# KELVIN-ASU/Lightweight-Multi-Modal-Scene-Understanding-via-Knowledge-Distillation

Hardware: AMD Instinct MI355X
Metric: PandaSet 2-class KD training frames/sec (higher is better)
Workload: dtype f32; 1 GPU; KD step: concat-fusion teacher fwd (eval) -> weighted-fusion student fwd/bwd (train BN), CE + T^2*KL(T=4) + feature-MSE, fused AdamW; random-init weights; teacher_fusion=concat, student_fusion=weighted, image=3x256x256, points_per_frame=80000, bev_grid=64x64, num_classes=2, per_gpu_batch=256, global_batch=256, parallelism=dp1

## Files before the change

### include/kd_hip.h

```cpp
#ifndef KD_HIP_H
#define KD_HIP_H
#include <stddef.h>
#include <stdint.h>

#ifdef __cplusplus
extern "C" {
#endif

#define KD_ACT_NONE 0
#define KD_ACT_RELU 1
#define KD_ACT_RELU6 2

int kd_version(void);
const char* kd_arch(void);
const char* kd_last_error_string(void);

int kd_set_gemm_split(int on);
int64_t kd_pwconv_stat_rows(int64_t M);
int64_t kd_pwconv_stat_rows_for(int64_t M, int K, int N, int pro, int epi, int with_addend);
int kd_set_gemm_stream(int mode);
int kd_pwconv_gemm(const float* A, int64_t lda, const float* A2, int64_t lda2, int pro, int pro_act,
                   const float* p0, const float* p1, const float* p2, const float* p3, const float* p4,
                   const float* W, const float* bias, float* C, int64_t ldc, const float* addend,
                   int64_t ldadd, int epi, const float* X, int64_t ldx, const float* esc, const float* esh,
// ... 149 lines not shown
int64_t kd_lidar_seg_stat_rows(int64_t ncells);
int kd_lidar_seg_max_bwd(const float* y, const float* sc, const float* sh, int act, const float* grid,
                         const float* dout, const float* mean, const float* invstd, const int* seg_start,
                         const int* perm, const int* row_of_point, float* G, float* partial, int64_t P,
                         int64_t ncells, int C, void* stream);
int kd_lidar_compact(const float* pts, float* out_pts, int* out_cell, int* counter, int B, int64_t N, int H, int W,
                     float x0, float x1, float y0, float y1, void* stream);
int kd_lidar_scatter_max_idx_fwd(const float* y, const float* sc, const float* sh, int act, const int* cell_idx,
                                 float* grid, int64_t P, int C, int64_t ncells, const int* p_dev, void* stream);

int kd_bilinear_accum_fwd(const float* in, const float* sc, const float* sh, int act, float* out, int accumulate,
                          int B, int Hi, int Wi, int Ho, int Wo, int C, void* stream);
int kd_bilinear_sum_fwd(const float* in0, const float* sc0, const float* sh0, int act0, int H0, int W0, const float* in1,
                        const float* sc1, const float* sh1, int act1, int H1, int W1, const float* in2, const float* sc2,
                        const float* sh2, int act2, int H2, int W2, float* out, int B, int Ho, int Wo, int C, void* stream);
int kd_bilinear_bwd(const float* dout, const float* in, const float* sc, const float* sh, int act,
                    const float* mean, const float* invstd, float* gin, float* partial, int B, int Hi, int Wi,
                    int Ho, int Wo, int C, void* stream);
int kd_weighted_fuse_fwd(const float* cat, const float* sc, const float* sh, const float* hraw, const float* w2,
                         const float* b2, float* out, float* wts, int64_t M, int C, void* stream);
size_t kd_weighted_fuse_bwd_ws_bytes(int64_t M, int C);
int kd_weighted_fuse_bwd(const float* dout, const float* cat, const float* sc, const float* sh, const float* hraw,
                         const float* w2, const float* wts, float* dcat, float* gh, float* dparams, int64_t M,
                         int C, void* ws, size_t ws_bytes, void* stream);
int kd_cls_conv_fwd(const float* x, const float* sc, const float* sh, int act, const float* w, const float* b,
                    float* logits_nchw, int64_t M, int HW, int Cin, int NC, void* stream);
size_t kd_cls_conv_bwd_ws_bytes(int64_t M, int Cin, int NC);
int64_t kd_cls_conv_bwd_stat_rows(int64_t M, int Cin);
int kd_cls_conv_bwd(const float* dlog_nchw, const float* x, const float* sc, const float* sh, int act,
                    const float* mean, const float* invstd, const float* w, float* gx, float* partial, float* dwb,
                    int64_t M, int HW, int Cin, int NC, void* ws, size_t ws_bytes, void* stream);

int64_t kd_deconv_stat_rows(int64_t npix_out, int Cout);
int kd_deconv4x4s2_col2im_fwd(const float* col, float* out, float* partial, int B, int H, int W, int Cout,
                             void* stream);
int kd_deconv4x4s2_im2col_bwd(const float* D, const float* Y, const float* al, const float* be, const float* ga,
                             const float* msc, const float* msh, int act, float* dcol, int B, int H, int W,
                             int Cout, void* stream);
int kd_cls3x3_fwd(const float* x, const float* sc, const float* sh, int act, const float* w, const float* b,
                  float* logits_nchw, int B, int H, int W, int Cin, int NC, void* stream);
int64_t kd_cls3x3_bwd_stat_rows(int64_t npix, int Cin);
size_t kd_cls3x3_bwd_ws_bytes(int64_t npix, int Cin, int NC);
int kd_cls3x3_bwd(const float* dlog_nchw, const float* x, const float* sc, const float* sh, int act,
                  const float* mean, const float* invstd, const float* w, float* gx, float* partial, float* dwb,
                  int B, int H, int W, int Cin, int NC, void* ws, size_t ws_bytes, void* stream);

size_t kd_bev_rasterize_ws_bytes(int B, int H, int W);
int kd_bev_rasterize(const float* x, const float* y, const int64_t* cls, const int64_t* offsets, int B, int64_t n_total,
                     int remap, uint64_t remap_bits, int H, int W, float x_min, float x_span, float x_max, float y_min,
                     float y_span, float y_max, void* ws, size_t ws_bytes, int64_t* mask, void* stream);
int kd_semantic_remap(const int64_t* raw, int64_t n, uint64_t remap_bits, int64_t* out, void* stream);
int kd_points_prepare(const float* x, const float* y, const float* z, const float* intensity, const int64_t* choice,
                      int64_t n, int64_t max_points, float* out, void* stream);
int kd_image_u8hwc_to_f32chw(const uint8_t* in, float* out, int H, int W, void* stream);
int kd_image_u8hwc_to_f32chw_batch(const uint8_t* in, float* out, int B, int H, int W, void* stream);
int kd_points_prepare_batch(const float* x, const float* y, const float* z, const float* intensity, const int64_t* offsets,
                            const uint64_t* frame_keys, int B, int64_t n_total, int64_t max_points, uint64_t seed, float* out,
                            void* stream);

size_t kd_seg_loss_ws_bytes(int64_t npix);
int kd_seg_loss_fwd_bwd(const float* zs, const float* zt, const int64_t* target, const float* class_w,
                        int ignore_index, float T, float alpha, float gscale, const float* gscale_dev, float* losses,
                        float* dzs, int B, int NC, int HW, void* ws, size_t ws_bytes, void* stream);
size_t kd_mse_ws_bytes(int64_t n);
int kd_mse_fwd_bwd(const float* a, const float* b, int64_t n, float gcoef, const float* gscale_dev, float* loss,
                   float* da, void* ws, size_t ws_bytes, void* stream);
int kd_kd_total(const float* ce_kl, const float* mse_c, const float* mse_l, float ckl, float beta, float* total, void* stream);
int64_t kd_mse_slab_blocks(int64_t n);
int kd_mse_partial(const float* a, const float* b, int64_t n, float gcoef, float* da, float* slab, void* stream);
int kd_kd_objective_final(const float* ce_kl, const float* slab_c, int64_t n_c, const float* slab_l, int64_t n_l, float ckl, float beta,
                          float* out, void* stream);
int kd_argmax_confusion(const float* logits, const int64_t* target, int ignore_index, uint64_t* conf,
                        int64_t* pred, int B, int NC, int M, int HW, void* stream);
int kd_adamw_step(float* p, const float* g, float* m, float* v, int64_t n, float lr, float beta1, float beta2,
                  float eps, float weight_decay, int step, float ginv, void* stream);
int kd_adamw_step_dev(float* p, const float* g, float* m, float* v, int64_t n, float* state, float beta1,
                      float beta2, float eps, float weight_decay, float ginv, void* stream);

int kd_dw_pw_infer_supported(int Ch, int Cout, int stride);
int kd_dw_pw_infer(const float* x, const float* isc, const float* ish, int iact, const float* wd, const float* dsc, const float* dsh,
                   int dact, const float* wp, const float* pbias, const float* psc, const float* psh, int pact, const float* res,
                   int64_t ldres, float* out, int64_t ldo, int B, int H, int W, int Ch, int stride, int Cout, void* stream);

int kd_bf16_stem(const float* x_nchw, const float* w, const float* sc, const float* sh, int act, void* y, int B, int Cin, int H,
                 int W, int Cout, void* stream);
int kd_bf16_dwconv3x3(const void* x, const float* w, const float* sc, const float* sh, int act, void* y, int B, int H, int W,
                      int C, int stride, void* stream);
int kd_bf16_pwconv(const void* A, int64_t lda, int a_kind, const float* W, const float* bias, const float* esc, const float* esh,
                   int act, void* C, int64_t ldc, const void* res, int64_t ldres, int epi, int64_t M, int K, int N,
                   const int* m_dev, const float* l0w, const float* l0b, const float* sc0, const float* sh0, int act0,
                   const int* cell, float* grid, int64_t ldgrid, void* stream);
int kd_bf16_bilinear_sum(const void* in0, int H0, int W0, const void* in1, int H1, int W1, const void* in2, int H2, int W2,
                         void* out, int B, int Ho, int Wo, int C, void* stream);
int kd_bf16_cls_conv(const void* x, const float* w, const float* b, float* logits_nchw, int64_t M, int HW, int Cin, int NC,
                     void* stream);
int kd_bf16_weighted_tail(const void* h, const void* cat, const float* w2, const float* b2, void* out, int64_t M, int C,
                          void* stream);

#ifdef __cplusplus
}
#endif
#endif
```

### lightweight-multi-modal-scene-understanding-via-knowledge-distillation_amd/csrc/kd_block.hip

```cpp
#include "kd_gemm_args.h"

namespace {

struct DwPwArgs {
  const float* x; const float* isc; const float* ish; int iact;
  const float* wd;
  const float* dsc; const float* dsh; int dact;
  const float* wp; const float* pbias;
  const float* psc; const float* psh; int pact;
  const float* res; int64_t ldres;
  float* out; int64_t ldo;
  int B, H, W, Ch, Ho, Wo;
  int tiles_x, tiles_y;
};

constexpr int NTHR = 256, KC = 32, CQN = KC / 4;
constexpr int XLD = KC + 4;
__device__ __forceinline__ int sw_off(int row, int chunk) { return (chunk ^ ((row >> 2) & 3)) * 8; }

template <int STRIDE, int NCB>
__global__ __launch_bounds__(NTHR, 2) void dw_pw_infer_kernel(DwPwArgs a) {
  constexpr int TH = 8, TW = STRIDE == 1 ? 16 : 8, MT = TH * TW, NRB = MT / 32;
  constexpr int HT = (TH - 1) * STRIDE + 3, WT = (TW - 1) * STRIDE + 3, HP = HT * WT;
  constexpr int COUT = 32 * NCB;
  constexpr int NH = (HP * CQN + NTHR - 1) / NTHR;
  constexpr int NJG = (NTHR / 64) / NRB;
  constexpr int NBW = NCB >= NJG ? NCB / NJG : 1;
  extern __shared__ __attribute__((aligned(16))) unsigned char smem_raw[];
  float* Xs = reinterpret_cast<float*>(smem_raw);
  unsigned short* Ap = reinterpret_cast<unsigned short*>(smem_raw + (size_t)HP * XLD * 4);
  unsigned short* Wp = Ap + 3 * MT * KC;
  const int tid = threadIdx.x, lane = tid & 63, wave = tid >> 6;
  const int r = lane & 31, h = lane >> 5;

  int t = blockIdx.x;
  const int tx0 = (t % a.tiles_x) * TW; t /= a.tiles_x;
  const int ty0 = (t % a.tiles_y) * TH;
  const int b = t / a.tiles_y;
  const int iy0 = ty0 * STRIDE - 1, ix0 = tx0 * STRIDE - 1;
  const int cq = tid & (CQN - 1);
  const int pl = tid / CQN;
  const bool deferred = a.isc != nullptr;

  const int rb = wave % NRB;
  const int jb0 = (wave / NRB) * NBW;
  const bool mma = jb0 < NCB;
  f32x16 acc[NBW];
#pragma unroll
  for (int j = 0; j < NBW; ++j)
#pragma unroll
    for (int q = 0; q < 16; ++q) acc[j][q] = 0.f;

  float4 xh[NH], wr[NCB], wt[9], isc = make_float4(1.f, 1.f, 1.f, 1.f), ish = kd_zero4(), dsc, dsh;
  auto issue = [&](int k0) {
#pragma unroll
    for (int i = 0; i < NH; ++i) {
      int e = tid + NTHR * i;
      e = e < HP * CQN ? e : HP * CQN - 1;
      const int hp = e / CQN;
      int iy = iy0 + hp / WT, ix = ix0 + hp % WT;
      iy = iy < 0 ? 0 : (iy >= a.H ? a.H - 1 : iy);
      ix = ix < 0 ? 0 : (ix >= a.W ? a.W - 1 : ix);
      xh[i] = kd_ld4(a.x + (((int64_t)b * a.H + iy) * a.W + ix) * a.Ch + k0 + 4 * cq);
    }
#pragma unroll
    for (int i = 0; i < NCB; ++i) wr[i] = kd_ld4(a.wp + (int64_t)(pl + 32 * i) * a.Ch + k0 + 4 * cq);
#pragma unroll
    for (int i = 0; i < 9; ++i) wt[i] = kd_ld4(a.wd + (int64_t)(k0 + 4 * cq) * 9 + 4 * i);
    if (deferred) { isc = kd_ld4(a.isc + k0 + 4 * cq); ish = kd_ld4(a.ish + k0 + 4 * cq); }
    dsc = kd_ld4(a.dsc + k0 + 4 * cq); dsh = kd_ld4(a.dsh + k0 + 4 * cq);
  };

  issue(0);
  for (int k0 = 0; k0 < a.Ch; k0 += KC) {
#pragma unroll
    for (int i = 0; i < NH; ++i) {
      const int e = tid + NTHR * i;
      const int hp = (e < HP * CQN ? e : HP * CQN - 1) / CQN;
      const int iy = iy0 + hp / WT, ix = ix0 + hp % WT;
      const bool ok = iy >= 0 && iy < a.H && ix >= 0 && ix < a.W;
      float4 v = xh[i];
      if (deferred) v = kd_affine_act4(v, isc, ish, a.iact);
      v = make_float4(ok ? v.x : 0.f, ok ? v.y : 0.f, ok ? v.z : 0.f, ok ? v.w : 0.f);
      if (e < HP * CQN) kd_st4(Xs + hp * XLD + 4 * cq, v);
    }
#pragma unroll
    for (int i = 0; i < NCB; ++i) {
      const int n = pl + 32 * i;
      uint2 hi, mid, lo;
      kd_split3(wr[i], hi, mid, lo);
      unsigned short* d = Wp + n * KC + sw_off(n, cq >> 1) + (cq & 1) * 4;
      *reinterpret_cast<uint2*>(d) = hi;
      *reinterpret_cast<uint2*>(d + COUT * KC) = mid;
      *reinterpret_cast<uint2*>(d + 2 * COUT * KC) = lo;
    }
    float w9[4][9];
    {
      const float flat[36] = {wt[0].x, wt[0].y, wt[0].z, wt[0].w, wt[1].x, wt[1].y, wt[1].z, wt[1].w, wt[2].x, wt[2].y, wt[2].z, wt[2].w,
                              wt[3].x, wt[3].y, wt[3].z, wt[3].w, wt[4].x, wt[4].y, wt[4].z, wt[4].w, wt[5].x, wt[5].y, wt[5].z, wt[5].w,
                              wt[6].x, wt[6].y, wt[6].z, wt[6].w, wt[7].x, wt[7].y, wt[7].z, wt[7].w, wt[8].x, wt[8].y, wt[8].z, wt[8].w};
#pragma unroll
      for (int j = 0; j < 4; ++j)
#pragma unroll
        for (int tp = 0; tp < 9; ++tp) w9[j][tp] = flat[j * 9 + tp];
    }
    const float4 csc = dsc, csh = dsh;
    kd_lds_barrier();
    if (k0 + KC < a.Ch) issue(k0 + KC);

#pragma unroll
    for (int p = 0; p < MT / 32; ++p) {
      const int px = p * 32 + pl;
      const int ty = px / TW, tx = px % TW;
      const float* xp = Xs + ((ty * STRIDE) * WT + tx * STRIDE) * XLD + 4 * cq;
      float4 v = kd_zero4();
#pragma unroll
      for (int kh = 0; kh < 3; ++kh) {
        const float4 l = kd_ld4(xp + (kh * WT + 0) * XLD), c = kd_ld4(xp + (kh * WT + 1) * XLD), rr = kd_ld4(xp + (kh * WT + 2) * XLD);
        v.x = fmaf(l.x, w9[0][kh * 3], fmaf(c.x, w9[0][kh * 3 + 1], fmaf(rr.x, w9[0][kh * 3 + 2], v.x)));
        v.y = fmaf(l.y, w9[1][kh * 3], fmaf(c.y, w9[1][kh * 3 + 1], fmaf(rr.y, w9[1][kh * 3 + 2], v.y)));
        v.z = fmaf(l.z, w9[2][kh * 3], fmaf(c.z, w9[2][kh * 3 + 1], fmaf(rr.z, w9[2][kh * 3 + 2], v.z)));
        v.w = fmaf(l.w, w9[3][kh * 3], fmaf(c.w, w9[3][kh * 3 + 1], fmaf(rr.w, w9[3][kh * 3 + 2], v.w)));
      }
      v = kd_affine_act4(v, csc, csh, a.dact);
      uint2 hi, mid, lo;
      kd_split3(v, hi, mid, lo);
      unsigned short* d = Ap + px * KC + sw_off(px, cq >> 1) + (cq & 1) * 4;
      *reinterpret_cast<uint2*>(d) = hi;
      *reinterpret_cast<uint2*>(d + MT * KC) = mid;
      *reinterpret_cast<uint2*>(d + 2 * MT * KC) = lo;
    }
    kd_lds_barrier();

    if (mma) {
#pragma unroll
      for (int ks = 0; ks < KC / 16; ++ks) {
        const int ko = sw_off(r, ks * 2 + h);
        bf16x8 fa[3], fb[NBW][3];
#pragma unroll
        for (int p = 0; p < 3; ++p) {
          fa[p] = *reinterpret_cast<const bf16x8*>(Ap + (p * MT + rb * 32 + r) * KC + ko);
#pragma unroll
          for (int j = 0; j < NBW; ++j) fb[j][p] = *reinterpret_cast<const bf16x8*>(Wp + (p * COUT + (jb0 + j) * 32 + r) * KC + ko);
        }
        constexpr int PA[6] = {0, 2, 1, 0, 1, 0}, PB[6] = {2, 0, 1, 1, 0, 0};
#pragma unroll
        for (int tt = 0; tt < 6; ++tt)
#pragma unroll
          for (int j = 0; j < NBW; ++j) acc[j] = __builtin_amdgcn_mfma_f32_32x32x16_bf16(fa[PA[tt]], fb[j][PB[tt]], acc[j], 0, 0, 0);
      }
    }
    kd_lds_barrier();
  }

  if (!mma) return;
#pragma unroll
  for (int j = 0; j < NBW; ++j) {
    const int col = (jb0 + j) * 32 + r;
    const float bias = a.pbias ? a.pbias[col] : 0.f, esc = a.psc[col], esh = a.psh[col];
#pragma unroll
    for (int q = 0; q < 16; ++q) {
      const int px = rb * 32 + (q & 3) + 8 * (q >> 2) + 4 * h;
      const int oy = ty0 + px / TW, ox = tx0 + px % TW;
      if (oy < a.Ho && ox < a.Wo) {
        const int64_t m = ((int64_t)b * a.Ho + oy) * a.Wo + ox;
        float v = kd_act(kd_affine(acc[j][q] + bias, esc, esh), a.pact);
        if (a.res) v += a.res[m * a.ldres + col];
        a.out[m * a.ldo + col] = v;
      }
    }
  }
}

template <int STRIDE, int NCB>
int launch(const DwPwArgs& a, hipStream_t st) {
  constexpr int TH = 8, TW = STRIDE == 1 ? 16 : 8, MT = TH * TW;
  constexpr int HP = ((TH - 1) * STRIDE + 3) * ((TW - 1) * STRIDE + 3);
  constexpr size_t lds = (size_t)HP * XLD * 4 + (size_t)3 * MT * KC * 2 + (size_t)3 * NCB * 32 * KC * 2;
  static_assert(lds <= 160 * 1024, "the staged tiles must fit the LDS of one CU");
  static std::atomic<uint64_t> lds_raised{0};
  const hipError_t e = kd_raise_dynamic_lds((const void*)dw_pw_infer_kernel<STRIDE, NCB>, lds, lds_raised);
  KD_REQUIRE(e == hipSuccess, (int)e, "kd_dw_pw_infer: cannot raise the dynamic LDS limit to %zu B: %s", lds, hipGetErrorString(e));
  const int64_t grid = (int64_t)a.B * a.tiles_y * a.tiles_x;
  hipLaunchKernelGGL((dw_pw_infer_kernel<STRIDE, NCB>), dim3((unsigned)grid), dim3(NTHR), lds, st, a);
  return kd_check_launch("kd_dw_pw_infer");
}

}

extern "C" {

int kd_dw_pw_infer_supported(int Ch, int Cout, int stride) {
  if (Ch < 32 || Ch % 32 != 0) return 0;
  if (stride == 1) return Cout == 32 || Cout == 64;
  if (stride == 2) return Cout == 64;
  return 0;
}

int kd_dw_pw_infer(const float* x, const float* isc, const float* ish, int iact, const float* wd, const float* dsc, const float* dsh,
                   int dact, const float* wp, const float* pbias, const float* psc, const float* psh, int pact, const float* res,
                   int64_t ldres, float* out, int64_t ldo, int B, int H, int W, int Ch, int stride, int Cout, void* stream) {
  KD_REQUIRE(x && wd && dsc && dsh && wp && psc && psh && out && B > 0 && H > 0 && W > 0, KD_ERR_ARG, "kd_dw_pw_infer: bad args");
  KD_REQUIRE(!isc || ish, KD_ERR_ARG, "kd_dw_pw_infer: isc needs ish");
  KD_REQUIRE(kd_dw_pw_infer_supported(Ch, Cout, stride), KD_ERR_SHAPE, "kd_dw_pw_infer: no instance for Ch=%d Cout=%d stride=%d", Ch, Cout, stride);
  KD_REQUIRE(ldo >= Cout && (!res || ldres >= Cout), KD_ERR_SHAPE, "kd_dw_pw_infer: row strides smaller than Cout");
  KD_REQUIRE(kd_aligned16(x) && kd_aligned16(wd) && kd_aligned16(wp) && kd_aligned16(dsc) && kd_aligned16(dsh) && kd_aligned16(isc) &&
             kd_aligned16(ish), KD_ERR_ALIGN, "kd_dw_pw_infer: 16-byte alignment");
  const int Ho = (H - 1) / stride + 1, Wo = (W - 1) / stride + 1;
  KD_REQUIRE((int64_t)B * Ho * Wo < ((int64_t)1 << 31), KD_ERR_SHAPE, "kd_dw_pw_infer: too many output pixels");
  const int TH = 8, TW = stride == 1 ? 16 : 8;
  DwPwArgs a{x, isc, ish, iact, wd, dsc, dsh, dact, wp, pbias, psc, psh, pact, res, ldres, out, ldo, B, H, W, Ch, Ho, Wo,
             (Wo + TW - 1) / TW, (Ho + TH - 1) / TH};
  hipStream_t st = (hipStream_t)stream;
  if (stride == 1) {
    if (Cout == 32) return launch<1, 1>(a, st);
    return launch<1, 2>(a, st);
  }
  return launch<2, 2>(a, st);
}

}
```

### lightweight-multi-modal-scene-understanding-via-knowledge-distillation_amd/kdrt/units.py

```python
from __future__ import annotations

import os
from typing import List, Optional, Sequence

import torch

from . import gradsink, ops
from .lib import KDError, lib
from .ops import ACT_NONE, ACT_RELU, BNC, Operand, P, ld, stream


ENCODER_WIDTHS = (8, 16, 24, 32, 40)


def check_encoder_width(base_channels: int) -> None:
    if base_channels not in ENCODER_WIDTHS:
        raise KDError(f"TwinLiteEncoder(base_channels={base_channels}) is not supported: base_channels must be one of "
                      f"{', '.join(map(str, ENCODER_WIDTHS))} (a multiple of 8, at most 40)")


class UnitSpec:

    def __init__(self, kind: str, conv, bn, act: int):
        self.kind, self.conv, self.bn, self.act = kind, conv, bn, act
# ... 118 lines not shown
            return Operand(None, rec.out_geom, rec.bnc, spec.act, virt=(pts, w, b)), rec
    elif kind == "ct":
        B, H, W = inp.geom
        Cin, Cout = w.shape[0], w.shape[1]
        if tuple(w.shape[2:]) != (4, 4) or inp.C != Cin:
            raise KDError(f"transposed conv expects a [{inp.C}, Cout, 4, 4] weight, got {tuple(w.shape)}")
        dev = inp.raw.device
        Wf = ops.transpose(w.view(Cin, Cout * 16))
        col = torch.empty(inp.M, Cout * 16, device=dev, dtype=torch.float32)
        ops.pw_gemm(inp.raw, Wf, col, M=inp.M, K=Cin, N=Cout * 16, pro=1 if inp.bnc is not None else 0, pro_act=inp.act,
                    p=(inp.sc, inp.sh, None, None, None), epi=0)
        Mo = B * 4 * H * W
        y = torch.empty(Mo, Cout, device=dev, dtype=torch.float32)
        partial, rows = None, 0
        if training:
            rows = lib.kd_deconv_stat_rows(Mo, Cout)
            partial = torch.empty(rows * 2 * Cout, device=dev, dtype=torch.float32)
        lib.call("kd_deconv4x4s2_col2im_fwd", P(col), P(y), P(partial), B, H, W, Cout, stream())
        rec.out_geom = (B, 2 * H, 2 * W)
        rec.bnc = _coeffs(spec, partial, rows, Cout, Mo, training, bnc, dev)
    else:
        raise KDError(f"unknown unit kind {kind}")
    rec.y = y
    return Operand(y, rec.out_geom, rec.bnc, spec.act), rec


def run_mode(training: bool) -> int:
    return 1 if training else (0 if torch.is_grad_enabled() else 2)


def inference_tail_ok(units, infer: bool) -> bool:
    return infer and len(units) > 0 and units[-1].kind == "pw"


def pw_forward_final(spec: UnitSpec, inp: Operand, res: Optional[torch.Tensor] = None) -> torch.Tensor:
    w, b = spec.conv.weight, spec.conv.bias
    N, K = w.shape[0], w.shape[1]
    if inp.C != K:
        raise KDError(f"pointwise conv expects {K} input channels, got {inp.C}")
    dev = w.device
    bnc = _coeffs(spec, None, 0, N, inp.M, False, None, dev)
    y = torch.empty(inp.M, N, device=dev, dtype=torch.float32)
    ops.pw_gemm(inp.raw, w, y, M=inp.M, K=K, N=N, pro=1 if inp.bnc is not None else 0, pro_act=inp.act,
                p=(inp.sc, inp.sh, None, None, None), bias=b, addend=res, epi=5, esc=bnc.scale, esh=bnc.shift,
                epi_act=spec.act)
    return y


DW_PW_FUSED = [1]


def dw_pw_tail_ok(units, cur: Operand) -> bool:
    mode = DW_PW_FUSED[0]
    if mode == 0 or len(units) < 2 or units[-2].kind != "dw" or units[-1].kind != "pw":
        return False
    if ops.get_gemm_arithmetic() != "split" or not isinstance(cur, Operand):
        return False
    if ld(cur.raw) != cur.C:
        return False
    dwu, pwu = units[-2], units[-1]
    Ch, Cout = dwu.conv.weight.shape[0], pwu.conv.weight.shape[0]
    if not lib.kd_dw_pw_infer_supported(Ch, Cout, dwu.stride):
        return False
    return mode >= 2 or (Cout == 64 and Ch >= 192)


def dw_pw_forward_final(dwu: UnitSpec, pwu: UnitSpec, inp: Operand, res: Optional[torch.Tensor] = None):
    B, H, W = inp.geom
    Ch, Cout = inp.C, pwu.conv.weight.shape[0]
    if dwu.conv.weight.shape[0] != Ch or pwu.conv.weight.shape[1] != Ch:
        raise KDError(f"depthwise / pointwise pair expects {dwu.conv.weight.shape[0]} channels, got {Ch}")
    s = dwu.stride
    Ho, Wo = (H - 1) // s + 1, (W - 1) // s + 1
    dev = inp.raw.device
    bd = _coeffs(dwu, None, 0, Ch, B * Ho * Wo, False, None, dev)
    bp = _coeffs(pwu, None, 0, Cout, B * Ho * Wo, False, None, dev)
    out = torch.empty(B * Ho * Wo, Cout, device=dev, dtype=torch.float32)
    lib.call("kd_dw_pw_infer", P(inp.raw), P(inp.sc), P(inp.sh), inp.act, P(dwu.conv.weight), P(bd.scale), P(bd.shift), dwu.act,
             P(pwu.conv.weight), P(pwu.conv.bias), P(bp.scale), P(bp.shift), pwu.act, P(res), ld(res) if res is not None else 0,
             P(out), Cout, B, H, W, Ch, s, Cout, stream())
    return out, (B, Ho, Wo)


def infer_tail(units, cur, res: Optional[torch.Tensor] = None):
    n_head = len(units) - 2
    if n_head >= 0:
        head = cur
        for u in units[:n_head]:
            head, _ = unit_forward(u, head, False)
        if dw_pw_tail_ok(units, head):
            return dw_pw_forward_final(units[-2], units[-1], head, res)
        cur = head
        units = units[n_head:]
    for u in units[:-1]:
        cur, _ = unit_forward(u, cur, False)
    return pw_forward_final(units[-1], cur, res), cur.geom


def unit_backward(rec: _Rec, g, need_input_grad: bool = True, addend: Optional[torch.Tensor] = None):
    spec = rec.spec
    y, bnc = rec.y, rec.bnc
    M, C = y.shape if y is not None else (rec.inp.shape[0], rec.w.shape[0])
    out_op = Operand(y, rec.out_geom, bnc, spec.act)
    pstride = None
    if g[0] == "D":
        t = g[1]
        partial, rows = ops.bn_bwd_reduce(t, out_op)
        msc, msh, mact = bnc.scale, bnc.shift, spec.act
        if mact == ACT_NONE:
            msc = msh = None
    else:
        t, partial, rows = g[1], g[2], g[3]
        pstride = g[4] if len(g) > 4 else None
        msc, msh, mact = None, None, ACT_NONE
    tables = g[0] == "GS"
    if tables and not (spec.kind == "pw" and rec.inp.virt is None and rec.inp.bnc is not None):
        raise KDError("table-form scatter gradient needs a pointwise unit with a deferred input")
    beta_p = spec.bn.bias
    g_buf, g_dir = gradsink.out_for(rec.gamma)
    b_buf, b_dir = gradsink.out_for(beta_p)
    want_dbias = spec.has_bias and spec.kind != "l0"
    cb_buf, cb_dir = gradsink.out_for(rec.b) if want_dbias else (None, False)
    dgamma, dbeta, abg, dbias = ops.bn_bwd_finalize(partial, rows, C, M, rec.gamma, bnc, rec.training,
                                                    want_dbias=want_dbias, pstride=pstride, dgamma=g_buf, dbeta=b_buf,
                                                    dbias=cb_buf)
    al, be, ga = abg[0], abg[1], abg[2]
    dev = rec.w.device
    kind = spec.kind
    g_in = None
    if kind == "pw":
        inp = rec.inp
        N, K = C, inp.C
        dW, w_dir = gradsink.out_for(rec.w)
        fused = (tables and need_input_grad and addend is None and lib.kd_lidar_l2_bwd_supported(N, K)
                 and ld(y) == N and ld(inp.raw) == K)
        fused1 = (inp.virt is not None and need_input_grad and addend is None and not tables
                  and mact == ACT_NONE and inp.act == ACT_RELU and lib.kd_lidar_l1_bwd_supported(N, K) and ld(t) == N and ld(y) == N)
        if fused or fused1:
            pass
        elif tables:
            ops.l2_wgrad(t, out_op, dW, inp=inp, al=al, be=be, ga=ga)
        elif inp.virt is not None:
            ops.l1_wgrad(t, y, dW, op=inp, al=al, be=be, ga=ga, msc=msc, msh=msh, mact=mact)
        else:
            ops.pw_wgrad(t, inp.raw, dW, M=M, N=N, K=K, X=y, d_mode=2, d_act=mact, al=al, be=be, ga=ga, msc=msc, msh=msh,
                         a_mode=1 if inp.bnc is not None else 0, a_act=inp.act, asc=inp.sc, ash=inp.sh)
        if need_input_grad:
            Wt = ops.transpose(rec.w.view(N, K), owner=rec.w)
            if fused1:
                rows_in = lib.kd_lidar_l1_bwd_stat_rows(M)
                part_in = torch.empty(rows_in * 2 * K, device=dev, dtype=torch.float32)
                m1 = torch.empty(4, K, device=dev, dtype=torch.float32)
                ops.l1_bwd(t, y, Wt, dW, op=inp, al=al, be=be, ga=ga, partial=part_in, partial_rows=rows_in, moments=m1)
                g_in = ("GM", m1, part_in, rows_in)
            elif inp.virt is not None:
                if addend is not None:
                    raise KDError("addend on a virtual LiDAR layer-0 input is not supported")
                rows_in = lib.kd_lidar_l1_dgrad_stat_rows(M, N, K)
                part_in = torch.empty(rows_in * 2 * K, device=dev, dtype=torch.float32)
                m1 = torch.empty(4, K, device=dev, dtype=torch.float32)
                ops.l1_dgrad(t, y, Wt, None, op=inp, al=al, be=be, ga=ga, msc=msc, msh=msh, mact=mact, partial=part_in,
                             partial_rows=rows_in, moments=m1)
                g_in = ("GM", m1, part_in, rows_in)
            elif fused:
                gin = torch.empty(M, K, device=dev, dtype=torch.float32)
                rows_in = lib.kd_lidar_l2_bwd_stat_rows(M)
                part_in = torch.empty(rows_in * 2 * K, device=dev, dtype=torch.float32)
# ... 790 lines not shown
```

Measured before the change: 3524 frames/s.

## Fuse expand-pw, depthwise and project-pw into one teacher inference block kernel

```diff
diff --git a/include/kd_hip.h b/include/kd_hip.h
--- a/include/kd_hip.h
+++ b/include/kd_hip.h
@@ -255,6 +255,12 @@
                    int dact, const float* wp, const float* pbias, const float* psc, const float* psh, int pact, const float* res,
                    int64_t ldres, float* out, int64_t ldo, int B, int H, int W, int Ch, int stride, int Cout, void* stream);
 
+int kd_block_infer_supported(int Cin, int Ch, int Cout, int stride);
+int kd_block_infer(const float* x, const float* we, const float* ebias, const float* esc, const float* esh, int eact, const float* wd,
+                   const float* dsc, const float* dsh, int dact, const float* wp, const float* pbias, const float* psc, const float* psh,
+                   int pact, const float* res, int64_t ldres, float* out, int64_t ldo, int B, int H, int W, int Cin, int Ch, int stride,
+                   int Cout, void* stream);
+
 int kd_bf16_stem(const float* x_nchw, const float* w, const float* sc, const float* sh, int act, void* y, int B, int Cin, int H,
                  int W, int Cout, void* stream);
 int kd_bf16_dwconv3x3(const void* x, const float* w, const float* sc, const float* sh, int act, void* y, int B, int H, int W,
diff --git a/lightweight-multi-modal-scene-understanding-via-knowledge-distillation_amd/csrc/kd_block.hip b/lightweight-multi-modal-scene-understanding-via-knowledge-distillation_amd/csrc/kd_block.hip
--- a/lightweight-multi-modal-scene-understanding-via-knowledge-distillation_amd/csrc/kd_block.hip
+++ b/lightweight-multi-modal-scene-understanding-via-knowledge-distillation_amd/csrc/kd_block.hip
@@ -17,6 +17,101 @@
 constexpr int NTHR = 256, KC = 32, CQN = KC / 4;
 constexpr int XLD = KC + 4;
 __device__ __forceinline__ int sw_off(int row, int chunk) { return (chunk ^ ((row >> 2) & 3)) * 8; }
+
+template <int NCB>
+__device__ __forceinline__ void stage_wp(unsigned short* Wp, const float4 (&wr)[NCB], int pl, int cq) {
+  constexpr int COUT = 32 * NCB;
+#pragma unroll
+  for (int i = 0; i < NCB; ++i) {
+    const int n = pl + 32 * i;
+    uint2 hi, mid, lo;
+    kd_split3(wr[i], hi, mid, lo);
+    unsigned short* d = Wp + n * KC + sw_off(n, cq >> 1) + (cq & 1) * 4;
+    *reinterpret_cast<uint2*>(d) = hi;
+    *reinterpret_cast<uint2*>(d + COUT * KC) = mid;
+    *reinterpret_cast<uint2*>(d + 2 * COUT * KC) = lo;
+  }
+}
+
+__device__ __forceinline__ void taps_of(const float4 (&wt)[9], float (&w9)[4][9]) {
+  const float flat[36] = {wt[0].x, wt[0].y, wt[0].z, wt[0].w, wt[1].x, wt[1].y, wt[1].z, wt[1].w, wt[2].x, wt[2].y, wt[2].z, wt[2].w,
+                          wt[3].x, wt[3].y, wt[3].z, wt[3].w, wt[4].x, wt[4].y, wt[4].z, wt[4].w, wt[5].x, wt[5].y, wt[5].z, wt[5].w,
+                          wt[6].x, wt[6].y, wt[6].z, wt[6].w, wt[7].x, wt[7].y, wt[7].z, wt[7].w, wt[8].x, wt[8].y, wt[8].z, wt[8].w};
+#pragma unroll
+  for (int j = 0; j < 4; ++j)
+#pragma unroll
+    for (int tp = 0; tp < 9; ++tp) w9[j][tp] = flat[j * 9 + tp];
+}
+
+template <int STRIDE>
+__device__ __forceinline__ void dw_phase(const float* Xs, unsigned short* Ap, const float (&w9)[4][9], float4 csc, float4 csh, int dact,
+                                         int pl, int cq) {
+  constexpr int TH = 8, TW = STRIDE == 1 ? 16 : 8, MT = TH * TW, WT = (TW - 1) * STRIDE + 3;
+#pragma unroll
+  for (int p = 0; p < MT / 32; ++p) {
+    const int px = p * 32 + pl;
+    const int ty = px / TW, tx = px % TW;
+    const float* xp = Xs + ((ty * STRIDE) * WT + tx * STRIDE) * XLD + 4 * cq;
+    float4 v = kd_zero4();
+#pragma unroll
+    for (int kh = 0; kh < 3; ++kh) {
+      const float4 l = kd_ld4(xp + (kh * WT + 0) * XLD), c = kd_ld4(xp + (kh * WT + 1) * XLD), rr = kd_ld4(xp + (kh * WT + 2) * XLD);
+      v.x = fmaf(l.x, w9[0][kh * 3], fmaf(c.x, w9[0][kh * 3 + 1], fmaf(rr.x, w9[0][kh * 3 + 2], v.x)));
+      v.y = fmaf(l.y, w9[1][kh * 3], fmaf(c.y, w9[1][kh * 3 + 1], fmaf(rr.y, w9[1][kh * 3 + 2], v.y)));
+      v.z = fmaf(l.z, w9[2][kh * 3], fmaf(c.z, w9[2][kh * 3 + 1], fmaf(rr.z, w9[2][kh * 3 + 2], v.z)));
+      v.w = fmaf(l.w, w9[3][kh * 3], fmaf(c.w, w9[3][kh * 3 + 1], fmaf(rr.w, w9[3][kh * 3 + 2], v.w)));
+    }
+    v = kd_affine_act4(v, csc, csh, dact);
+    uint2 hi, mid, lo;
+    kd_split3(v, hi, mid, lo);
+    unsigned short* d = Ap + px * KC + sw_off(px, cq >> 1) + (cq & 1) * 4;
+    *reinterpret_cast<uint2*>(d) = hi;
+    *reinterpret_cast<uint2*>(d + MT * KC) = mid;
+    *reinterpret_cast<uint2*>(d + 2 * MT * KC) = lo;
+  }
+}
+
+constexpr int TSN = KC * 9 + 2 * KC;
+constexpr int PA[6] = {0, 2, 1, 0, 1, 0}, PB[6] = {2, 0, 1, 1, 0, 0};
+
+template <int MT, int COUT, int NBW>
+__device__ __forceinline__ void project_chunk(const unsigned short* Ap, const unsigned short* Wp, f32x16 (&acc)[NBW], int rb, int jb0, int r, int h) {
+#pragma unroll
+  for (int ks = 0; ks < KC / 16; ++ks) {
+    const int ko = sw_off(r, ks * 2 + h);
+    bf16x8 fa[3], fb[NBW][3];
+#pragma unroll
+    for (int p = 0; p < 3; ++p) {
+      fa[p] = *reinterpret_cast<const bf16x8*>(Ap + (p * MT + rb * 32 + r) * KC + ko);
+#pragma unroll
+      for (int j = 0; j < NBW; ++j) fb[j][p] = *reinterpret_cast<const bf16x8*>(Wp + (p * COUT + (jb0 + j) * 32 + r) * KC + ko);
+    }
+#pragma unroll
+    for (int tt = 0; tt < 6; ++tt)
+#pragma unroll
+      for (int j = 0; j < NBW; ++j) acc[j] = __builtin_amdgcn_mfma_f32_32x32x16_bf16(fa[PA[tt]], fb[j][PB[tt]], acc[j], 0, 0, 0);
+  }
+}
+
+template <int TW, int NBW>
+__device__ __forceinline__ void tail_epilogue(const DwPwArgs& a, const f32x16 (&acc)[NBW], int b, int ty0, int tx0, int rb, int jb0, int r, int h) {
+#pragma unroll
+  for (int j = 0; j < NBW; ++j) {
+    const int col = (jb0 + j) * 32 + r;
+    const float bias = a.pbias ? a.pbias[col] : 0.f, esc = a.psc[col], esh = a.psh[col];
+#pragma unroll
+    for (int q = 0; q < 16; ++q) {
+      const int px = rb * 32 + (q & 3) + 8 * (q >> 2) + 4 * h;
+      const int oy = ty0 + px / TW, ox = tx0 + px % TW;
+      if (oy < a.Ho && ox < a.Wo) {
+        const int64_t m = ((int64_t)b * a.Ho + oy) * a.Wo + ox;
+        float v = kd_act(kd_affine(acc[j][q] + bias, esc, esh), a.pact);
+        if (a.res) v += a.res[m * a.ldres + col];
+        a.out[m * a.ldo + col] = v;
+      }
+    }
+  }
+}
 
 template <int STRIDE, int NCB>
 __global__ __launch_bounds__(NTHR, 2) void dw_pw_infer_kernel(DwPwArgs a) {
@@ -84,92 +179,21 @@
       v = make_float4(ok ? v.x : 0.f, ok ? v.y : 0.f, ok ? v.z : 0.f, ok ? v.w : 0.f);
       if (e < HP * CQN) kd_st4(Xs + hp * XLD + 4 * cq, v);
     }
-#pragma unroll
-    for (int i = 0; i < NCB; ++i) {
-      const int n = pl + 32 * i;
-      uint2 hi, mid, lo;
-      kd_split3(wr[i], hi, mid, lo);
-      unsigned short* d = Wp + n * KC + sw_off(n, cq >> 1) + (cq & 1) * 4;
-      *reinterpret_cast<uint2*>(d) = hi;
-      *reinterpret_cast<uint2*>(d + COUT * KC) = mid;
-      *reinterpret_cast<uint2*>(d + 2 * COUT * KC) = lo;
-    }
+    stage_wp<NCB>(Wp, wr, pl, cq);
     float w9[4][9];
-    {
-      const float flat[36] = {wt[0].x, wt[0].y, wt[0].z, wt[0].w, wt[1].x, wt[1].y, wt[1].z, wt[1].w, wt[2].x, wt[2].y, wt[2].z, wt[2].w,
-                              wt[3].x, wt[3].y, wt[3].z, wt[3].w, wt[4].x, wt[4].y, wt[4].z, wt[4].w, wt[5].x, wt[5].y, wt[5].z, wt[5].w,
-                              wt[6].x, wt[6].y, wt[6].z, wt[6].w, wt[7].x, wt[7].y, wt[7].z, wt[7].w, wt[8].x, wt[8].y, wt[8].z, wt[8].w};
-#pragma unroll
-      for (int j = 0; j < 4; ++j)
-#pragma unroll
-        for (int tp = 0; tp < 9; ++tp) w9[j][tp] = flat[j * 9 + tp];
-    }
+    taps_of(wt, w9);
     const float4 csc = dsc, csh = dsh;
     kd_lds_barrier();
     if (k0 + KC < a.Ch) issue(k0 + KC);
 
-#pragma unroll
-    for (int p = 0; p < MT / 32; ++p) {
-      const int px = p * 32 + pl;
-      const int ty = px / TW, tx = px % TW;
-      const float* xp = Xs + ((ty * STRIDE) * WT + tx * STRIDE) * XLD + 4 * cq;
-      float4 v = kd_zero4();
-#pragma unroll
-      for (int kh = 0; kh < 3; ++kh) {
-        const float4 l = kd_ld4(xp + (kh * WT + 0) * XLD), c = kd_ld4(xp + (kh * WT + 1) * XLD), rr = kd_ld4(xp + (kh * WT + 2) * XLD);
-        v.x = fmaf(l.x, w9[0][kh * 3], fmaf(c.x, w9[0][kh * 3 + 1], fmaf(rr.x, w9[0][kh * 3 + 2], v.x)));
-        v.y = fmaf(l.y, w9[1][kh * 3], fmaf(c.y, w9[1][kh * 3 + 1], fmaf(rr.y, w9[1][kh * 3 + 2], v.y)));
-        v.z = fmaf(l.z, w9[2][kh * 3], fmaf(c.z, w9[2][kh * 3 + 1], fmaf(rr.z, w9[2][kh * 3 + 2], v.z)));
-        v.w = fmaf(l.w, w9[3][kh * 3], fmaf(c.w, w9[3][kh * 3 + 1], fmaf(rr.w, w9[3][kh * 3 + 2], v.w)));
-      }
-      v = kd_affine_act4(v, csc, csh, a.dact);
-      uint2 hi, mid, lo;
-      kd_split3(v, hi, mid, lo);
-      unsigned short* d = Ap + px * KC + sw_off(px, cq >> 1) + (cq & 1) * 4;
-      *reinterpret_cast<uint2*>(d) = hi;
-      *reinterpret_cast<uint2*>(d + MT * KC) = mid;
-      *reinterpret_cast<uint2*>(d + 2 * MT * KC) = lo;
-    }
+    dw_phase<STRIDE>(Xs, Ap, w9, csc, csh, a.dact, pl, cq);
     kd_lds_barrier();
 
-    if (mma) {
-#pragma unroll
-      for (int ks = 0; ks < KC / 16; ++ks) {
-        const int ko = sw_off(r, ks * 2 + h);
-        bf16x8 fa[3], fb[NBW][3];
-#pragma unroll
-        for (int p = 0; p < 3; ++p) {
-          fa[p] = *reinterpret_cast<const bf16x8*>(Ap + (p * MT + rb * 32 + r) * KC + ko);
-#pragma unroll
-          for (int j = 0; j < NBW; ++j) fb[j][p] = *reinterpret_cast<const bf16x8*>(Wp + (p * COUT + (jb0 + j) * 32 + r) * KC + ko);
-        }
-        constexpr int PA[6] = {0, 2, 1, 0, 1, 0}, PB[6] = {2, 0, 1, 1, 0, 0};
-#pragma unroll
-        for (int tt = 0; tt < 6; ++tt)
-#pragma unroll
-          for (int j = 0; j < NBW; ++j) acc[j] = __builtin_amdgcn_mfma_f32_32x32x16_bf16(fa[PA[tt]], fb[j][PB[tt]], acc[j], 0, 0, 0);
-      }
-    }
+    if (mma) project_chunk<MT, COUT, NBW>(Ap, Wp, acc, rb, jb0, r, h);
     kd_lds_barrier();
   }
 
-  if (!mma) return;
-#pragma unroll
-  for (int j = 0; j < NBW; ++j) {
-    const int col = (jb0 + j) * 32 + r;
-    const float bias = a.pbias ? a.pbias[col] : 0.f, esc = a.psc[col], esh = a.psh[col];
-#pragma unroll
-    for (int q = 0; q < 16; ++q) {
-      const int px = rb * 32 + (q & 3) + 8 * (q >> 2) + 4 * h;
-      const int oy = ty0 + px / TW, ox = tx0 + px % TW;
-      if (oy < a.Ho && ox < a.Wo) {
-        const int64_t m = ((int64_t)b * a.Ho + oy) * a.Wo + ox;
-        float v = kd_act(kd_affine(acc[j][q] + bias, esc, esh), a.pact);
-        if (a.res) v += a.res[m * a.ldres + col];
-        a.out[m * a.ldo + col] = v;
-      }
-    }
-  }
+  if (mma) tail_epilogue<TW, NBW>(a, acc, b, ty0, tx0, rb, jb0, r, h);
 }
 
 template <int STRIDE, int NCB>
@@ -184,6 +208,195 @@
   const int64_t grid = (int64_t)a.B * a.tiles_y * a.tiles_x;
   hipLaunchKernelGGL((dw_pw_infer_kernel<STRIDE, NCB>), dim3((unsigned)grid), dim3(NTHR), lds, st, a);
   return kd_check_launch("kd_dw_pw_infer");
+}
+
+struct BlockArgs {
+  DwPwArgs d;
+  const float* we; const float* ebias;
+};
+
+template <int CIN>
+__device__ __forceinline__ int we_off(int n, int chunk) {
+  static_assert(CIN == 32 || CIN == 64, "expand-weight rows of 64 or 128 bytes");
+  return (chunk ^ (CIN == 32 ? (n >> 2) & 3 : (n >> 1) & 7)) * 8;
+}
+
+template <int STRIDE, int CKB, int NCB>
+__global__ __launch_bounds__(NTHR, 2) void block_infer_kernel(BlockArgs g) {
+  constexpr int TH = 8, TW = STRIDE == 1 ? 16 : 8, MT = TH * TW, NRB = MT / 32;
+  constexpr int HT = (TH - 1) * STRIDE + 3, WT = (TW - 1) * STRIDE + 3, HP = HT * WT;
+  constexpr int CIN = 32 * CKB, COUT = 32 * NCB;
+  constexpr int NJG = (NTHR / 64) / NRB;
+  constexpr int NBW = NCB >= NJG ? NCB / NJG : 1;
+  constexpr int NXB = (HP + 31) / 32, XBW = (NXB + 3) / 4;
+  constexpr int NKS = CIN / 16;
+  const DwPwArgs& a = g.d;
+  extern __shared__ __attribute__((aligned(16))) unsigned char smem_raw[];
+  float* Xs = reinterpret_cast<float*>(smem_raw);
+  unsigned short* Ap = reinterpret_cast<unsigned short*>(smem_raw + (size_t)NXB * 32 * XLD * 4);
+  unsigned short* Wp = Ap + 3 * MT * KC;
+  unsigned short* We = Wp + 3 * COUT * KC;
+  float* Ts = reinterpret_cast<float*>(We + 3 * KC * CIN);
+  const int tid = threadIdx.x, lane = tid & 63, wave = tid >> 6;
+  const int r = lane & 31, h = lane >> 5;
+
+  int t = blockIdx.x;
+  const int tx0 = (t % a.tiles_x) * TW; t /= a.tiles_x;
+  const int ty0 = (t % a.tiles_y) * TH;
+  const int b = t / a.tiles_y;
+  const int iy0 = ty0 * STRIDE - 1, ix0 = tx0 * STRIDE - 1;
+  const int cq = tid & (CQN - 1);
+  const int pl = tid / CQN;
+  const int rb = wave % NRB;
+  const int jb0 = (wave / NRB) * NBW;
+  const bool mma = jb0 < NCB;
+  f32x16 acc[NBW];
+#pragma unroll
+  for (int j = 0; j < NBW; ++j)
+#pragma unroll
+    for (int q = 0; q < 16; ++q) acc[j][q] = 0.f;
+
+  float4 wr[NCB], wx[CKB], tp = kd_zero4();
+  float ebn = 0.f, escn, eshn;
+  auto issue_e = [&](int k0) {
+#pragma unroll
+    for (int i = 0; i < CKB; ++i) wx[i] = kd_ld4(g.we + (int64_t)(k0 + pl) * CIN + 32 * i + 4 * cq);
+    if (g.ebias) ebn = g.ebias[k0 + r];
+    escn = a.isc[k0 + r]; eshn = a.ish[k0 + r];
+    if (tid < TSN / 4) {
+      const float* src = tid < 72 ? a.wd + (int64_t)k0 * 9 + 4 * tid : (tid < 80 ? a.dsc + k0 + 4 * (tid - 72) : a.dsh + k0 + 4 * (tid - 80));
+      tp = kd_ld4(src);
+    }
+  };
+  auto issue = [&](int k0) {
+#pragma unroll
+    for (int i = 0; i < NCB; ++i) wr[i] = kd_ld4(a.wp + (int64_t)(pl + 32 * i) * a.Ch + k0 + 4 * cq);
+    issue_e(k0 + KC < a.Ch ? k0 + KC : k0);
+  };
+  auto stage_ts = [&](int buf) { if (tid < TSN / 4) kd_st4(Ts + buf * TSN + 4 * tid, tp); };
+  auto stage_we = [&]() {
+#pragma unroll
+    for (int i = 0; i < CKB; ++i) {
+      const int k4 = 8 * i + cq;
+      uint2 hi, mid, lo;
+      kd_split3(wx[i], hi, mid, lo);
+      unsigned short* d = We + pl * CIN + we_off<CIN>(pl, k4 >> 1) + (k4 & 1) * 4;
+      *reinterpret_cast<uint2*>(d) = hi;
+      *reinterpret_cast<uint2*>(d + KC * CIN) = mid;
+      *reinterpret_cast<uint2*>(d + 2 * KC * CIN) = lo;
+    }
+  };
+
+  issue_e(0);
+  bf16x8 xf[XBW][NKS][3];
+  unsigned inm[XBW];
+  {
+    float4 xr[XBW][NKS][2];
+#pragma unroll
+    for (int i = 0; i < XBW; ++i) {
+      int hp = (wave + 4 * i) * 32 + r;
+      hp = hp < HP ? hp : HP - 1;
+      int iy = iy0 + hp / WT, ix = ix0 + hp % WT;
+      iy = iy < 0 ? 0 : (iy >= a.H ? a.H - 1 : iy);
+      ix = ix < 0 ? 0 : (ix >= a.W ? a.W - 1 : ix);
+      const float* xp = a.x + (((int64_t)b * a.H + iy) * a.W + ix) * CIN + 8 * h;
+#pragma unroll
+      for (int u = 0; u < NKS; ++u) { xr[i][u][0] = kd_ld4(xp + 16 * u); xr[i][u][1] = kd_ld4(xp + 16 * u + 4); }
+      inm[i] = 0;
+#pragma unroll
+      for (int q = 0; q < 16; ++q) {
+        const int row = (wave + 4 * i) * 32 + (q & 3) + 8 * (q >> 2) + 4 * h;
+        const int y = iy0 + row / WT, x = ix0 + row % WT;
+        inm[i] |= ((y >= 0 && y < a.H && x >= 0 && x < a.W) ? 1u : 0u) << q;
+      }
+    }
+    stage_we();
+    stage_ts(0);
+#pragma unroll
+    for (int i = 0; i < XBW; ++i)
+#pragma unroll
+      for (int u = 0; u < NKS; ++u) {
+        typedef __attribute__((ext_vector_type(4))) uint32_t u32x4;
+        uint2 h0, m0, l0, h1, m1, l1;
+        kd_split3(xr[i][u][0], h0, m0, l0);
+        kd_split3(xr[i][u][1], h1, m1, l1);
+        const u32x4 ph = {h0.x, h0.y, h1.x, h1.y}, pm = {m0.x, m0.y, m1.x, m1.y}, pq = {l0.x, l0.y, l1.x, l1.y};
+        xf[i][u][0] = __builtin_bit_cast(bf16x8, ph);
+        xf[i][u][1] = __builtin_bit_cast(bf16x8, pm);
+        xf[i][u][2] = __builtin_bit_cast(bf16x8, pq);
+      }
+  }
+  kd_lds_barrier();
+
+  for (int k0 = 0;; k0 += KC) {
+    const bool more = k0 < a.Ch;
+    const float eb = ebn, esc = escn, esh = eshn;
+    if (k0 > 0 && mma) project_chunk<MT, COUT, NBW>(Ap, Wp, acc, rb, jb0, r, h);
+    if (!more) break;
+    issue(k0);
+    const float4 eb4 = make_float4(eb, eb, eb, eb), esc4 = make_float4(esc, esc, esc, esc), esh4 = make_float4(esh, esh, esh, esh);
+#pragma unroll
+    for (int i = 0; i < XBW; ++i) {
+      if (wave + 4 * i < NXB) {
+        f32x16 e;
+#pragma unroll
+        for (int q = 0; q < 16; ++q) e[q] = 0.f;
+#pragma unroll
+        for (int u = 0; u < NKS; ++u) {
+          bf16x8 fb[3];
+#pragma unroll
+          for (int p = 0; p < 3; ++p) fb[p] = *reinterpret_cast<const bf16x8*>(We + (p * KC + r) * CIN + we_off<CIN>(r, 2 * u + h));
+#pragma unroll
+          for (int tt = 0; tt < 6; ++tt) e = __builtin_amdgcn_mfma_f32_32x32x16_bf16(xf[i][u][PA[tt]], fb[PB[tt]], e, 0, 0, 0);
+        }
+        float* xd = Xs + ((wave + 4 * i) * 32 + 4 * h) * XLD + r;
+#pragma unroll
+        for (int qg = 0; qg < 4; ++qg) {
+          float4 v = make_float4(e[4 * qg] + eb4.x, e[4 * qg + 1] + eb4.y, e[4 * qg + 2] + eb4.z, e[4 * qg + 3] + eb4.w);
+          v = kd_affine_act4(v, esc4, esh4, a.iact);
+          const float o[4] = {v.x, v.y, v.z, v.w};
+#pragma unroll
+          for (int qq = 0; qq < 4; ++qq) {
+            const int q = 4 * qg + qq;
+            xd[((q & 3) + 8 * (q >> 2)) * XLD] = ((inm[i] >> q) & 1u) ? o[qq] : 0.f;
+          }
+        }
+      }
+    }
+    kd_lds_barrier();
+
+    const int cb = (k0 / KC) & 1;
+    stage_wp<NCB>(Wp, wr, pl, cq);
+    stage_we();
+    stage_ts(cb ^ 1);
+    {
+      const float* tq = Ts + cb * TSN;
+      float4 wt[9];
+#pragma unroll
+      for (int i = 0; i < 9; ++i) wt[i] = kd_ld4(tq + 36 * cq + 4 * i);
+      float w9[4][9];
+      taps_of(wt, w9);
+      dw_phase<STRIDE>(Xs, Ap, w9, kd_ld4(tq + 288 + 4 * cq), kd_ld4(tq + 320 + 4 * cq), a.dact, pl, cq);
+    }
+    kd_lds_barrier();
+  }
+
+  if (mma) tail_epilogue<TW, NBW>(a, acc, b, ty0, tx0, rb, jb0, r, h);
+}
+
+template <int STRIDE, int CKB, int NCB>
+int launch_block(const BlockArgs& g, hipStream_t st) {
+  constexpr int TH = 8, TW = STRIDE == 1 ? 16 : 8, MT = TH * TW;
+  constexpr int HP = ((TH - 1) * STRIDE + 3) * ((TW - 1) * STRIDE + 3);
+  constexpr size_t lds = (size_t)((HP + 31) / 32 * 32) * XLD * 4 + (size_t)3 * MT * KC * 2 + (size_t)3 * NCB * 32 * KC * 2 +
+                         (size_t)3 * KC * CKB * 32 * 2 + (size_t)2 * TSN * 4;
+  static_assert(2 * lds <= 160 * 1024, "two workgroups share the LDS of one CU");
+  static std::atomic<uint64_t> lds_raised{0};
+  const hipError_t e = kd_raise_dynamic_lds((const void*)block_infer_kernel<STRIDE, CKB, NCB>, lds, lds_raised);
+  KD_REQUIRE(e == hipSuccess, (int)e, "kd_block_infer: cannot raise the dynamic LDS limit to %zu B: %s", lds, hipGetErrorString(e));
+  const int64_t grid = (int64_t)g.d.B * g.d.tiles_y * g.d.tiles_x;
+  hipLaunchKernelGGL((block_infer_kernel<STRIDE, CKB, NCB>), dim3((unsigned)grid), dim3(NTHR), lds, st, g);
+  return kd_check_launch("kd_block_infer");
 }
 
 }
@@ -219,4 +432,32 @@
   return launch<2, 2>(a, st);
 }
 
-}
+int kd_block_infer_supported(int Cin, int Ch, int Cout, int stride) {
+  if (Ch < 32 || Ch % 32 != 0) return 0;
+  if (stride == 1) return Cin == 64 && Cout == 64;
+  if (stride == 2) return Cin == 32 && Cout == 64;
+  return 0;
+}
+
+int kd_block_infer(const float* x, const float* we, const float* ebias, const float* esc, const float* esh, int eact, const float* wd,
+                   const float* dsc, const float* dsh, int dact, const float* wp, const float* pbias, const float* psc, const float* psh,
+                   int pact, const float* res, int64_t ldres, float* out, int64_t ldo, int B, int H, int W, int Cin, int Ch, int stride,
+                   int Cout, void* stream) {
+  KD_REQUIRE(x && we && esc && esh && wd && dsc && dsh && wp && psc && psh && out && B > 0 && H > 0 && W > 0, KD_ERR_ARG,
+             "kd_block_infer: bad args");
+  KD_REQUIRE(kd_block_infer_supported(Cin, Ch, Cout, stride), KD_ERR_SHAPE, "kd_block_infer: no instance for Cin=%d Ch=%d Cout=%d stride=%d",
+             Cin, Ch, Cout, stride);
+  KD_REQUIRE(ldo >= Cout && (!res || ldres >= Cout), KD_ERR_SHAPE, "kd_block_infer: row strides smaller than Cout");
+  KD_REQUIRE(kd_aligned16(x) && kd_aligned16(we) && kd_aligned16(wd) && kd_aligned16(wp) && kd_aligned16(dsc) && kd_aligned16(dsh),
+             KD_ERR_ALIGN, "kd_block_infer: 16-byte alignment");
+  const int Ho = (H - 1) / stride + 1, Wo = (W - 1) / stride + 1;
+  KD_REQUIRE((int64_t)B * Ho * Wo < ((int64_t)1 << 31), KD_ERR_SHAPE, "kd_block_infer: too many output pixels");
+  const int TH = 8, TW = stride == 1 ? 16 : 8;
+  BlockArgs g{{x, esc, esh, eact, wd, dsc, dsh, dact, wp, pbias, psc, psh, pact, res, ldres, out, ldo, B, H, W, Ch, Ho, Wo,
+               (Wo + TW - 1) / TW, (Ho + TH - 1) / TH}, we, ebias};
+  hipStream_t st = (hipStream_t)stream;
+  if (stride == 1) return launch_block<1, 2, 2>(g, st);
+  return launch_block<2, 1, 2>(g, st);
+}
+
+}
diff --git a/lightweight-multi-modal-scene-understanding-via-knowledge-distillation_amd/kdrt/units.py b/lightweight-multi-modal-scene-understanding-via-knowledge-distillation_amd/kdrt/units.py
--- a/lightweight-multi-modal-scene-understanding-via-knowledge-distillation_amd/kdrt/units.py
+++ b/lightweight-multi-modal-scene-understanding-via-knowledge-distillation_amd/kdrt/units.py
@@ -224,7 +224,49 @@
     return out, (B, Ho, Wo)
 
 
+BLOCK_INFER = [1]
+
+
+def block_infer_ok(units, cur) -> bool:
+    mode = BLOCK_INFER[0]
+    if mode == 0 or len(units) != 3 or [u.kind for u in units] != ["pw", "dw", "pw"]:
+        return False
+    if ops.get_gemm_arithmetic() != "split" or not isinstance(cur, Operand):
+        return False
+    if cur.bnc is not None or cur.raw is None or ld(cur.raw) != cur.C:
+        return False
+    eu, dwu, pwu = units
+    Ch, Cin = eu.conv.weight.shape[0], eu.conv.weight.shape[1]
+    Cout = pwu.conv.weight.shape[0]
+    if cur.C != Cin or dwu.conv.weight.shape[0] != Ch or pwu.conv.weight.shape[1] != Ch:
+        return False
+    if not lib.kd_block_infer_supported(Cin, Ch, Cout, dwu.stride):
+        return False
+    return mode >= 2 or (Cin, Ch, Cout, dwu.stride) in BLOCK_INFER_SHAPES
+
+
+BLOCK_INFER_SHAPES = {(32, 192, 64, 2), (64, 384, 64, 1)}
+
+
+def block_forward_final(eu: UnitSpec, dwu: UnitSpec, pwu: UnitSpec, inp: Operand, res: Optional[torch.Tensor] = None):
+    B, H, W = inp.geom
+    Cin, Ch, Cout = inp.C, eu.conv.weight.shape[0], pwu.conv.weight.shape[0]
+    s = dwu.stride
+    Ho, Wo = (H - 1) // s + 1, (W - 1) // s + 1
+    dev = inp.raw.device
+    be = _coeffs(eu, None, 0, Ch, inp.M, False, None, dev)
+    bd = _coeffs(dwu, None, 0, Ch, B * Ho * Wo, False, None, dev)
+    bp = _coeffs(pwu, None, 0, Cout, B * Ho * Wo, False, None, dev)
+    out = torch.empty(B * Ho * Wo, Cout, device=dev, dtype=torch.float32)
+    lib.call("kd_block_infer", P(inp.raw), P(eu.conv.weight), P(eu.conv.bias), P(be.scale), P(be.shift), eu.act, P(dwu.conv.weight),
+             P(bd.scale), P(bd.shift), dwu.act, P(pwu.conv.weight), P(pwu.conv.bias), P(bp.scale), P(bp.shift), pwu.act, P(res),
+             ld(res) if res is not None else 0, P(out), Cout, B, H, W, Cin, Ch, s, Cout, stream())
+    return out, (B, Ho, Wo)
+
+
 def infer_tail(units, cur, res: Optional[torch.Tensor] = None):
+    if block_infer_ok(units, cur):
+        return block_forward_final(units[0], units[1], units[2], cur, res)
     n_head = len(units) - 2
     if n_head >= 0:
         head = cur
```

After: 3568 frames/s, median of 6. +1.3%, better.
